# vita-epfl/CrowdNav

Hardware: AMD Instinct MI355X
Metric: env-steps/sec (whole node), 4096 envs x 5 humans, ORCA step (higher is better)
Workload: dtype f32 ORCA solve + f64 env step

## Files before the change

### crowdnav_amd/csrc/orca_device.h

```cpp
#pragma once
#include <hip/hip_runtime.h>

namespace cn {

constexpr int kWave = 64;
constexpr int kMaxNb = 10;
constexpr int kLineStride = kMaxNb + 1;
constexpr float kRvoEps = 0.00001f;
constexpr int kLazyCandFloat4 = (kWave / (kMaxNb - 1)) * ((kMaxNb - 1) + 4);

__device__ __forceinline__ void wave_lds_sync() {
    __builtin_amdgcn_fence(__ATOMIC_RELEASE, "wavefront");
    __builtin_amdgcn_wave_barrier();
    __builtin_amdgcn_fence(__ATOMIC_ACQUIRE, "wavefront");
}

__device__ __forceinline__ int opaque_tid() {
    int t = threadIdx.x;
    asm volatile("" : "+v"(t));
    return t;
}

struct OrcaParams {
    float neighbor_dist;
// ... 18 lines not shown
    const bool disc = overlap || (dot1 < 0.0f && dot1 * dot1 > rsum_sq * wlen_sq);
    const float root = sqrtf(disc ? wlen_sq : dist_sq - rsum_sq);
    const float inv = 1.0f / (disc ? root : dist_sq);
    const float nx = wx * inv, ny = wy * inv;
    const float kd = rsum * inv_t - root;
    const bool left = rpx * wy - rpy * wx > 0.0f;
    const float llx = (rpx * root - rpy * rsum) * inv, lly = (rpx * rsum + rpy * root) * inv;
    const float lrx = -((rpx * root + rpy * rsum) * inv), lry = -((-rpx * rsum + rpy * root) * inv);
    const float gx = left ? llx : lrx, gy = left ? lly : lry;
    const float dot2 = rvx * gx + rvy * gy;
    const float ldx = disc ? ny : gx;
    const float ldy = disc ? -nx : gy;
    const float ux = disc ? kd * nx : dot2 * gx - rvx;
    const float uy = disc ? kd * ny : dot2 * gy - rvy;
    return make_float4(svx + 0.5f * ux, svy + 0.5f * uy, ldx, ldy);
}

__device__ __forceinline__ void lp_start_point(float radius, float ox, float oy, float& rx, float& ry) {
    if (ox * ox + oy * oy > radius * radius) {
        const float inv = 1.0f / sqrtf(ox * ox + oy * oy);
        const float ux = ox * inv, uy = oy * inv;
        rx = ux * radius;
        ry = uy * radius;
    } else {
        rx = ox;
        ry = oy;
    }
}

template <int NJ>
__device__ __forceinline__ float4 lp_line_candidate(const float4 lk, const float4* prev, int k, float radius, float ox,
                                                    float oy, bool dir_opt) {
    const float px = lk.x, py = lk.y, dx = lk.z, dy = lk.w;
    const float dp = px * dx + py * dy;
    const float disc = (dp * dp + radius * radius) - (px * px + py * py);
    bool ok = !(disc < 0.0f);
    const float root = sqrtf(disc);
    float t_lo = -dp - root;
    float t_hi = -dp + root;
#pragma unroll
    for (int j = 0; j < NJ; ++j) {
        const float4 lj = prev[j];
        const bool use = j < k;
        const float den = dx * lj.w - dy * lj.z;
        const float num = lj.z * (py - lj.y) - lj.w * (px - lj.x);
        const bool parallel = fabsf(den) <= kRvoEps;
        const float t = num / den;
        ok = ok && !(use && parallel && num < 0.0f);
        const bool upper = use && !parallel && den >= 0.0f;
        const bool lower = use && !parallel && !(den >= 0.0f);
        t_hi = (upper && t < t_hi) ? t : t_hi;
        t_lo = (lower && t_lo < t) ? t : t_lo;
        ok = ok && !(t_lo > t_hi);
    }
    float t;
    if (dir_opt) {
        t = (ox * dx + oy * dy > 0.0f) ? t_hi : t_lo;
    } else {
        t = dx * (ox - px) + dy * (oy - py);
        t = (t < t_lo) ? t_lo : ((t > t_hi) ? t_hi : t);
    }
    return make_float4(px + t * dx, py + t * dy, ok ? 1.0f : 0.0f, 0.0f);
}

template <int MAXL>
__device__ __forceinline__ int lp_planar_scan(const float4* lines, const float4* cand, int n, float& rx, float& ry) {
    float4 lk[MAXL], ck[MAXL];
#pragma unroll
    for (int k = 0; k < MAXL; ++k) {
        lk[k] = lines[k];
        ck[k] = cand[k];
    }
    int fail = n;
#pragma unroll
    for (int k = 0; k < MAXL; ++k) {
        const float det = lk[k].z * (lk[k].y - ry) - lk[k].w * (lk[k].x - rx);
        const bool viol = (k < fail) & (det > 0.0f);
        const bool feasible = ck[k].z != 0.0f;
        rx = (viol & feasible) ? ck[k].x : rx;
        ry = (viol & feasible) ? ck[k].y : ry;
        fail = (viol & !feasible) ? k : fail;
    }
    return fail;
}

__device__ __forceinline__ int lp3_program_of(int m) { return m >= 6 ? 4 : (m >= 3 ? 3 : (m >= 1 ? 2 : 1)); }

__device__ __forceinline__ float4 lp3_project(const float4 li, const float4 lj) {
    const float d = li.z * lj.w - li.w * lj.z;
    const bool par = fabsf(d) <= kRvoEps;
    const bool same_dir = li.z * lj.z + li.w * lj.w > 0.0f;
    const float t = (lj.z * (li.y - lj.y) - lj.w * (li.x - lj.x)) / d;
    const float qx = par ? 0.5f * (li.x + lj.x) : li.x + t * li.z;
    const float qy = par ? 0.5f * (li.y + lj.y) : li.y + t * li.w;
    const float ex = lj.z - li.z, ey = lj.w - li.w;
    const float inv = 1.0f / sqrtf(ex * ex + ey * ey);
    const bool skip = par && same_dir;
    return make_float4(skip ? 0.0f : qx, skip ? 0.0f : qy, skip ? 0.0f : ex * inv, skip ? 0.0f : ey * inv);
}

__device__ __forceinline__ void lp3_scan(const float4* lines, const float4* proj, const float4* cand, int n, int begin,
                                         float radius, float& rx, float& ry) {
    float distance = 0.0f;
    float4 li[5];
#pragma unroll
    for (int i = 0; i < 5; ++i) li[i] = lines[i];
#pragma unroll
    for (int i = 0; i < 5; ++i) {
        float4 pk[4], ck[4];
#pragma unroll
        for (int k = 0; k < i; ++k) {
            pk[k] = proj[i * (i - 1) / 2 + k];
            ck[k] = cand[i * (i - 1) / 2 + k];
        }
        const float viol_i = li[i].z * (li[i].y - ry) - li[i].w * (li[i].x - rx);
        const bool active = (i >= begin) & (i < n) & (viol_i > distance);
        float r2x = -li[i].w * radius, r2y = li[i].z * radius;
        bool failed = false;
#pragma unroll
        for (int k = 0; k < i; ++k) {
            const float det = pk[k].z * (pk[k].y - r2y) - pk[k].w * (pk[k].x - r2x);
            const bool viol = !failed & (det > 0.0f);
            const bool feasible = ck[k].z != 0.0f;
            r2x = (viol & feasible) ? ck[k].x : r2x;
            r2y = (viol & feasible) ? ck[k].y : r2y;
            failed = failed | (viol & !feasible);
        }
        rx = (active & !failed) ? r2x : rx;
        ry = (active & !failed) ? r2y : ry;
        const float pen = li[i].z * (li[i].y - ry) - li[i].w * (li[i].x - rx);
        distance = active ? pen : distance;
    }
}

__device__ __forceinline__ float4 lp3_inner_program(const float4* proj, const float4* cand, int i, const float4 li, float radius) {
    const int base = i * (i - 1) / 2;
    float4 pk[4], ck[4];
#pragma unroll
    for (int k = 0; k < 4; ++k) {
        const int slot = base + k < 10 ? base + k : 9;
        pk[k] = proj[slot];
        ck[k] = cand[slot];
    }
    float r2x = -li.w * radius, r2y = li.z * radius;
    bool failed = false;
#pragma unroll
    for (int k = 0; k < 4; ++k) {
        const float det = pk[k].z * (pk[k].y - r2y) - pk[k].w * (pk[k].x - r2x);
        const bool viol = (k < i) & !failed & (det > 0.0f);
        const bool feasible = ck[k].z != 0.0f;
        r2x = (viol & feasible) ? ck[k].x : r2x;
        r2y = (viol & feasible) ? ck[k].y : r2y;
        failed = failed | (viol & !feasible);
    }
    return make_float4(r2x, r2y, failed ? 1.0f : 0.0f, 0.0f);
}
__device__ __forceinline__ void lp3_outer_scan(const float4* lines, const float4* prog, int n, int begin, float radius,
                                               float& rx, float& ry) {
    float4 li[5], pg[5];
#pragma unroll
    for (int i = 0; i < 5; ++i) {
        li[i] = lines[i];
        pg[i] = prog[i];
    }
    pg[0] = make_float4(-li[0].w * radius, li[0].z * radius, 0.0f, 0.0f);
    float distance = 0.0f;
// ... 157 lines not shown
        const float radius = sol[a].z;
        const float4 my = (l < n) ? lines[a * kLineStride + l] : make_float4(0.f, 0.f, 0.f, 0.f);
        float rx = r0.x, ry = r0.y, distance = 0.0f;
        int icur = need ? begin : n;
        while (true) {
            const bool cond = l >= icur && l < n && (my.z * (my.y - ry) - my.w * (my.x - rx) > distance);
            const unsigned long long m = __ballot(cond);
            if (m == 0ull) break;
            const unsigned gm = (unsigned)(m >> gbase) & kField;
            const bool act = gm != 0u;
            const int i = act ? __ffs(gm) - 1 : 0;
            const float4 li = lines[a * kLineStride + i];
            const float d = li.z * my.w - li.w * my.z;
            const bool par = fabsf(d) <= kRvoEps;
            const bool same_dir = li.z * my.z + li.w * my.w > 0.0f;
            const float t = (my.z * (li.y - my.y) - my.w * (li.x - my.x)) / d;
            const float qx = par ? 0.5f * (li.x + my.x) : li.x + t * li.z;
            const float qy = par ? 0.5f * (li.y + my.y) : li.y + t * li.w;
            const float ex = my.z - li.z, ey = my.w - li.w;
            const float inv = 1.0f / sqrtf(ex * ex + ey * ey);
            const float pz = ex * inv, pw = ey * inv;
            const bool valid = act && l < i && !(par && same_dir);
            const float ox = -li.w, oy = li.z;
            float r2x = ox * radius, r2y = oy * radius;
            int cur2 = 0;
            bool failed = false;
            while (true) {
                const bool viol = valid && l >= cur2 && (pz * (qy - r2y) - pw * (qx - r2x) > 0.0f);
                const unsigned long long m2 = __ballot(viol);
                if (m2 == 0ull) break;
                const unsigned gm2 = (unsigned)(m2 >> gbase) & kField;
                const bool act2 = gm2 != 0u;
                const int k = act2 ? __ffs(gm2) - 1 : 0;
                const float kx = __shfl(qx, gbase + k), ky = __shfl(qy, gbase + k);
                const float kz = __shfl(pz, gbase + k), kw = __shfl(pw, gbase + k);
                const float den = kz * pw - kw * pz;
                const float num = pz * (ky - qy) - pw * (kx - qx);
                const bool parallel = fabsf(den) <= kRvoEps;
                const float tk = num / den;
                const bool mine = act2 && valid && l < k;
                const bool bad = mine && parallel && num < 0.0f;
                const float c_hi = (mine && !parallel && den >= 0.0f) ? tk : inf;
                const float c_lo = (mine && !parallel && !(den >= 0.0f)) ? tk : -inf;
                const unsigned badm = (unsigned)(__ballot(bad) >> gbase) & kField;
                const float dp = kx * kz + ky * kw;
                const float disc = (dp * dp + radius * radius) - (kx * kx + ky * ky);
                bool ok = !(disc < 0.0f) && badm == 0u;
                const float root = sqrtf(disc);
                float t_lo = -dp - root;
                float t_hi = -dp + root;
#pragma unroll
                for (int j = 0; j < MAXL - 1; ++j) {
                    const float hj = __shfl(c_hi, gbase + j);
                    const float lj = __shfl(c_lo, gbase + j);
                    t_hi = (hj < t_hi) ? hj : t_hi;
                    t_lo = (t_lo < lj) ? lj : t_lo;
                }
                ok = ok && !(t_lo > t_hi);
                const float tt = (ox * kz + oy * kw > 0.0f) ? t_hi : t_lo;
                if (act2) {
                    if (ok) {
                        r2x = kx + tt * kz;
                        r2y = ky + tt * kw;
                        cur2 = k + 1;
                    } else {
                        failed = true;
                        cur2 = MAXL;
                    }
                }
            }
            if (act) {
                if (!failed) {
                    rx = r2x;
                    ry = r2y;
                }
                distance = li.z * (li.y - ry) - li.w * (li.x - rx);
                icur = i + 1;
            }
        }
        if (need && l == 0) res[a] = make_float4(rx, ry, r0.z, 0.0f);
    }
}

__device__ __forceinline__ float4 lp_line_candidate_pairs5(const float4* lq, int k, int lane, float radius, float ox, float oy) {
    const float inf = __builtin_inff();
    const float4 lk = lq[k];
    const int row0 = k == 0 ? 4 : k, j0 = k == 0 ? 2 : 0;
    const int row1 = k == 0 ? 4 : (k == 1 ? 3 : k), j1 = k == 0 ? 3 : (k == 1 ? 2 : 1);
    const bool own0 = k != 0, own1 = k >= 2;
    const float4 K0 = lq[row0], J0 = lq[j0], K1 = lq[row1], J1 = lq[j1];
    float hi_c[2], lo_c[2];
    bool bad_c[2];
#pragma unroll
    for (int s = 0; s < 2; ++s) {
        const float4 K = s ? K1 : K0, J = s ? J1 : J0;
        const float den = K.z * J.w - K.w * J.z;
        const float num = J.z * (K.y - J.y) - J.w * (K.x - J.x);
        const bool parallel = fabsf(den) <= kRvoEps;
        const float t = num / den;
        bad_c[s] = parallel && num < 0.0f;
        hi_c[s] = (!parallel && den >= 0.0f) ? t : inf;
        lo_c[s] = (!parallel && !(den >= 0.0f)) ? t : -inf;
    }
    float hi_o = own0 ? hi_c[0] : inf, lo_o = own0 ? lo_c[0] : -inf;
    bool bad_o = own0 && bad_c[0];
    float hi_h = own0 ? inf : hi_c[0], lo_h = own0 ? -inf : lo_c[0];
    bool bad_h = !own0 && bad_c[0];
    hi_o = (own1 && hi_c[1] < hi_o) ? hi_c[1] : hi_o;
    lo_o = (own1 && lo_o < lo_c[1]) ? lo_c[1] : lo_o;
    bad_o = bad_o || (own1 && bad_c[1]);
    hi_h = (!own1 && hi_c[1] < hi_h) ? hi_c[1] : hi_h;
    lo_h = (!own1 && lo_h < lo_c[1]) ? lo_c[1] : lo_h;
    bad_h = bad_h || (!own1 && bad_c[1]);
    const int src = lane - (k == 3 ? 2 : (k == 4 ? 4 : 0));
    const float hi_r = __shfl(hi_h, src), lo_r = __shfl(lo_h, src);
    const int bad_r = __shfl(bad_h ? 1 : 0, src);
    const bool has = k >= 3;
    const float px = lk.x, py = lk.y, dx = lk.z, dy = lk.w;
    const float dp = px * dx + py * dy;
    const float disc = (dp * dp + radius * radius) - (px * px + py * py);
    bool ok = !(disc < 0.0f);
    const float root = sqrtf(disc);
    float t_lo = -dp - root;
    float t_hi = -dp + root;
    t_hi = (hi_o < t_hi) ? hi_o : t_hi;
    t_lo = (t_lo < lo_o) ? lo_o : t_lo;
    t_hi = (has && hi_r < t_hi) ? hi_r : t_hi;
    t_lo = (has && t_lo < lo_r) ? lo_r : t_lo;
    ok = ok && !bad_o && !(has && bad_r != 0) && !(t_lo > t_hi);
    float t = dx * (ox - px) + dy * (oy - py);
    t = (t < t_lo) ? t_lo : ((t > t_hi) ? t_hi : t);
    return make_float4(px + t * dx, py + t * dy, ok ? 1.0f : 0.0f, 0.0f);
}

__device__ __forceinline__ float4 lp_line_candidate_pairs9(const float4 lk, const float4* prow, float4* bpart, int l, bool live,
                                                           float radius, float ox, float oy) {
    const float px = lk.x, py = lk.y, dx = lk.z, dy = lk.w;
    const float dp = px * dx + py * dy;
    const float disc = (dp * dp + radius * radius) - (px * px + py * py);
    bool ok = !(disc < 0.0f);
    const float root = sqrtf(disc);
    float t_lo = -dp - root;
    float t_hi = -dp + root;
    const float inf = __builtin_inff();
    const bool helper = l < 4;
    const float4 hk = prow[helper ? 8 - l : l];
    float hi_own = inf, lo_own = -inf, hi_help = inf, lo_help = -inf;
    bool bad_own = false, bad_help = false;
#pragma unroll
    for (int s = 0; s < 4; ++s) {
        const bool own = !helper || s < l;
        const float4 lj = prow[own ? s : 4 + s - l];
        const float kx = own ? px : hk.x, ky = own ? py : hk.y, kdx = own ? dx : hk.z, kdy = own ? dy : hk.w;
        const float den = kdx * lj.w - kdy * lj.z;
        const float num = lj.z * (ky - lj.y) - lj.w * (kx - lj.x);
        const bool parallel = fabsf(den) <= kRvoEps;
        const float t = num / den;
        const bool bad = parallel && num < 0.0f;
        const bool upper = !parallel && den >= 0.0f;
        const bool lower = !parallel && !(den >= 0.0f);
        hi_own = (own && upper && t < hi_own) ? t : hi_own;
        lo_own = (own && lower && lo_own < t) ? t : lo_own;
        bad_own = bad_own || (own && bad);
        hi_help = (!own && upper && t < hi_help) ? t : hi_help;
        lo_help = (!own && lower && lo_help < t) ? t : lo_help;
        bad_help = bad_help || (!own && bad);
    }
    if (live && helper) bpart[3 - l] = make_float4(hi_help, lo_help, bad_help ? 1.0f : 0.0f, 0.0f);
    wave_lds_sync();
    const bool has_help = l >= 5;
    const float4 hb = bpart[has_help ? l - 5 : 0];
    t_hi = (hi_own < t_hi) ? hi_own : t_hi;
    t_lo = (t_lo < lo_own) ? lo_own : t_lo;
    t_hi = (has_help && hb.x < t_hi) ? hb.x : t_hi;
    t_lo = (has_help && t_lo < hb.y) ? hb.y : t_lo;
    ok = ok && !bad_own && !(has_help && hb.z != 0.0f) && !(t_lo > t_hi);
    const float t = (ox * dx + oy * dy > 0.0f) ? t_hi : t_lo;
    return make_float4(px + t * dx, py + t * dy, ok ? 1.0f : 0.0f, 0.0f);
}

template <int MAXL, bool GROUP_ROWS = false>
__device__ __forceinline__ void lp_relaxed_lazy(const float4* lines, float4* proj, float4* cand, const int* count,
                                                const float4* sol, float4* res, const int* todo, int n_todo, int threads) {
    constexpr int W = MAXL - 1, G = kWave / W;
    constexpr unsigned kField = (1u << W) - 1u;
    const int tid = opaque_tid();
    const int wl = tid & (kWave - 1);
    const int g = wl / W, l = wl - g * W;
    const int gbase = g * W;
    const int waves = (threads + kWave - 1) / kWave;
    float4* const crow = cand + ((tid / kWave) * G + (g < G ? g : 0)) * W;
    float4* const bpart = cand + (size_t)waves * G * W + ((tid / kWave) * G + (g < G ? g : 0)) * 4;
#ifdef CN_PHASE_TIMING
    unsigned long long pt_rounds = 0ull, pt_hand = 0ull;
    const unsigned long long pt_t0 = __builtin_readcyclecounter();
#endif
    for (int chunk = tid / kWave; chunk * G < n_todo; chunk += waves) {
        const int hand_end = waves == 1 ? n_todo : (chunk * G + G < n_todo ? chunk * G + G : n_todo);
        int next = chunk * G + G;
        bool live = false, need = false, tail = false;
        int a = 0, n = 0, icur = 0;
        float radius = 0.0f, rx = 0.0f, ry = 0.0f, r0z = 0.0f, distance = 0.0f;
        float4 my = make_float4(0.f, 0.f, 0.f, 0.f), last = my;
        float4* prow = proj;
        const auto take = [&](int idx) {
            live = g < G && idx < hand_end;
            a = live ? todo[idx] : 0;
            const float4 r0 = res[a];
            n = live ? count[a] : 0;
            const int begin = __float_as_int(r0.z);
            need = live && begin < n;
            radius = sol[a].z;
            my = (l < n) ? lines[a * kLineStride + l] : make_float4(0.f, 0.f, 0.f, 0.f);
            tail = l == W - 1 && W < n;
            last = tail ? lines[a * kLineStride + W] : make_float4(0.f, 0.f, 0.f, 0.f);
// ... 74 lines not shown
```

### crowdnav_amd/csrc/rollout_fused.h

```cpp
#pragma once
#include "rollout_kernels.h"

namespace cn {

constexpr int kFusedMaxNC = 5;

template <typename T>
__device__ __forceinline__ T in_vgpr(T x) {
    asm volatile("" : "+v"(x));
    return x;
}

__device__ __forceinline__ void stage_agent(const Params& P, const Smem& s, const Lane& L, const AgentRegs& r,
                                            double human_safety, float4* kin) {
    if (L.lane >= P.nA) return;
    kin[L.lane] = make_float4((float)r.px, (float)r.py, (float)r.vx, (float)r.vy);
    s.posd[L.lane] = make_double2(r.px, r.py);
    s.rad[L.lane] = r.rad;
    s.hview[L.lane] = (float)(r.rad + 0.01 + human_safety);
}

__device__ __forceinline__ void preferred_velocity(const AgentRegs& r, float max_speed, bool solve, float4& sol, float4& start) {
    const double gdx = r.gx - r.px, gdy = r.gy - r.py;
    const double speed = norm2(gdx, gdy);
    const float pref_x = (float)(speed > 1.0 ? gdx / speed : gdx);
    const float pref_y = (float)(speed > 1.0 ? gdy / speed : gdy);
    sol = make_float4(pref_x, pref_y, max_speed, solve ? 1.0f : 0.0f);
    float sx, sy;
    lp_start_point(max_speed, pref_x, pref_y, sx, sy);
    start = make_float4(sx, sy, 0.0f, 0.0f);
}

#define CN_FUSED_SYNC() wave_lds_sync()



struct PairRow {
    int my_info, my_slot, xbase;
};
__device__ __forceinline__ PairRow pair_row_of(const Params& P, const Smem& s, int lane) {
    PairRow pr{0, P.nA, 0};
    if (lane < P.pairs) {
        pr.my_info = s.pinfo[lane];
        const int c = (pr.my_info >> 16) & 0xff;
        pr.xbase = (lane - c) * 4;
        pr.my_slot = ((pr.my_info >> 24) & 1) ? ((pr.my_info >> 8) & 0xff) : P.nA;
    }
    return pr;
}

__device__ __forceinline__ float pair_rsum(const Smem& s, const PairRow& pr) {
    const int q = pr.my_info & 0xff, ol = (pr.my_info >> 8) & 0xff;
    const float* view = ((pr.my_info >> 25) & 1) ? s.rview : s.hview;
    return view[q] + view[ol];
}

template <typename Mid>
__device__ __forceinline__ void fused_pair_body(const Params& P, const Smem& s, const PairRow& pr, float range_sq, float rsum,
                                                const float4 me, const float4 other, Mid&& mid) {
    const int my_info = pr.my_info;
    const int q = my_info & 0xff, c = (my_info >> 16) & 0xff;
    const float odx = me.x - other.x, ody = me.y - other.y;
    const float mine = odx * odx + ody * ody;
    uint32_t vbk[kFusedMaxNC];
#pragma unroll
    for (int k = 0; k < kFusedMaxNC; ++k) {
        const uint32_t got = (uint32_t)__builtin_amdgcn_ds_bpermute(pr.xbase + 4 * k, (int)__float_as_uint(mine));
        vbk[k] = k < P.NC ? got : 0x7f800000u;
    }
    int rank = 0, within = 0;
    {
        const uint32_t mb = __float_as_uint(mine), rb = __float_as_uint(range_sq);
        uint32_t before = 0u, inside = 0u;
#pragma unroll
        for (int k = 0; k < kFusedMaxNC; ++k) {
            const uint32_t vb = vbk[k];
            const uint32_t tie = (uint32_t)(k - c) >> 31;
            before = __builtin_amdgcn_alignbit(before, vb - mb - tie, 31);
            inside = __builtin_amdgcn_alignbit(inside, vb - rb, 31);
        }
        within = __popc(inside);
        rank = __popc(before & inside);
    }
    mid();
    if (c == 0) s.count[q] = within < P.orca.max_neighbors ? within : P.orca.max_neighbors;
    if (mine < range_sq && rank < P.orca.max_neighbors)
        s.lines[q * kLineStride + rank] =
            make_half_plane(P.orca, me.x, me.y, me.z, me.w, other.x, other.y, other.z, other.w, rsum);
}
template <typename Mid>
__device__ __forceinline__ void fused_pair_phase(const Params& P, const Smem& s, const PairRow& pr, float range_sq, float rsum,
                                                 Mid&& mid) {
    const float4 me = s.kin[pr.my_info & 0xff];
    const float4 other = s.kin[pr.my_slot];
    fused_pair_body(P, s, pr, range_sq, rsum, me, other, mid);
}

template <int MAXL>
__device__ __forceinline__ void fused_candidates(const Params& P, const Smem& s, int lane) {
    if (lane < P.nA * MAXL) {
        const int q = lane / MAXL, k = lane - q * MAXL;
        const float4 so = s.sol[q];
        const float4* lq = s.lines + q * kLineStride;
        s.cand2[q * kLineStride + k] = lp_line_candidate_pairs5(lq, k, lane, so.z, so.x, so.y);
    }
}

__device__ __forceinline__ void split_barrier() {
    asm volatile("s_waitcnt lgkmcnt(0)\n\ts_barrier" ::: "memory");
}

struct Lp3Item {
    int a, m, i, base;
    bool item;
    float4 li, lj;
    float radius;
};
template <int MAXL>
__device__ __forceinline__ Lp3Item lp3_item_of(const Smem& s, int lane, unsigned long long mask) {
    constexpr int kPairs = MAXL * (MAXL - 1) / 2;
    Lp3Item it;
    const int t = lane / kPairs;
    it.m = lane - t * kPairs;
    it.a = 0;
    unsigned long long rest = mask;
#pragma unroll
    for (int u = 0; u < kWave / kPairs; ++u) {
        const int bit = rest ? __ffsll((long long)rest) - 1 : 0;
        it.a = (u == t) ? bit : it.a;
        rest &= rest - 1ull;
    }
    it.item = lane < (int)__popcll(mask) * kPairs;
    it.i = lp3_program_of(it.m), it.base = it.i * (it.i - 1) / 2;
    const float4* la = s.lines + it.a * kLineStride;
    it.li = la[it.i], it.lj = la[it.m - it.base];
    it.radius = s.sol[it.a].z;
    return it;
}
template <int MAXL>
__device__ __forceinline__ void lp3_head(const Smem& s, const Lp3Item& it) {
    const float4 pr = lp3_project(it.li, it.lj);
    if (it.item) s.proj[it.a * kLineStride + it.m] = pr;
    CN_FUSED_SYNC();
    if (it.item) {
        const float4* pa = s.proj + it.a * kLineStride + it.base;
        s.cand3[it.a * kLineStride + it.m] =
            lp_line_candidate<MAXL - 2>(pa[it.m - it.base], pa, it.m - it.base, it.radius, -it.li.w, it.li.z, true);
    }
}

template <int MAXL>
__device__ __forceinline__ bool split_has_head(unsigned int pred, int u, int n_steps) {
    return pred != 0u && __popc(pred) * (MAXL * (MAXL - 1) / 2) <= kWave && u < n_steps;
}

struct NoOp {
    __device__ __forceinline__ void operator()() const {}
};
template <int MAXL, int BASE_PRIO = 0, typename AfterScan = NoOp>
__device__ __forceinline__ unsigned long long fused_solve(const Params& P, const Smem& s, int lane, bool solve, float& rx,
                                                          float& ry, PhaseClock* clk, unsigned long long have = 0ull,
                                                          AfterScan&& after_scan = NoOp{}) {
    (void)P, (void)clk;
    rx = 0.0f, ry = 0.0f;
    int n = 0, fail = 0;
    if (solve) {
        n = s.count[lane];
        const float4 start = s.res[lane];
        rx = start.x, ry = start.y;
        fail = lp_planar_scan<MAXL>(s.lines + lane * kLineStride, s.cand2 + lane * kLineStride, n, rx, ry);
    }
    CN_TICK(clk, 3);
    const bool need = solve && fail < n;
    const unsigned long long nm = __ballot(need);
#ifdef CN_PHASE_TIMING
    if (clk) clk->acc[9] += __popcll(nm);
#endif
    after_scan();
    if (nm == 0ull) __builtin_amdgcn_s_setprio(BASE_PRIO);
    if (nm != 0ull) {
        __builtin_amdgcn_s_setprio(3);
        constexpr int kPairs = MAXL * (MAXL - 1) / 2;
        const int n_todo = __popcll(nm);
        bool one_pass_done = false;
        if (n_todo * kPairs <= kWave) {
            const Lp3Item it = lp3_item_of<MAXL>(s, lane, nm);
            const bool item = it.item;
            const int a = it.a, i = it.i, m = it.m, base = it.base;
            const float4 li = it.li;
            const float radius = it.radius;
            const bool hit = (nm & ~have) == 0ull;
            if (!hit) {
                lp3_head<MAXL>(s, it);
                CN_FUSED_SYNC();
            }
            if (item && m == base)
                s.cand2[a * kLineStride + i] = lp3_inner_program(s.proj + a * kLineStride, s.cand3 + a * kLineStride, i, li, radius);
            CN_FUSED_SYNC();
            if (need)
                lp3_outer_scan(s.lines + lane * kLineStride, s.cand2 + lane * kLineStride, n, fail, s.sol[lane].z, rx, ry);
            one_pass_done = true;
        } else {
            if (need) s.todo[__popcll(nm & ((1ull << lane) - 1ull))] = lane;
            CN_FUSED_SYNC();
            const int items = n_todo * kPairs;
            for (int p = lane; p < items; p += kWave) {
                const int t = p / kPairs, m = p - t * kPairs;
                const int a = s.todo[t];
                const int i = lp3_program_of(m), j = m - i * (i - 1) / 2;
                const float4* la = s.lines + a * kLineStride;
                s.proj[a * kLineStride + m] = lp3_project(la[i], la[j]);
            }
            CN_FUSED_SYNC();
            for (int p = lane; p < items; p += kWave) {
                const int t = p / kPairs, m = p - t * kPairs;
                const int a = s.todo[t];
                const int i = lp3_program_of(m), base = i * (i - 1) / 2;
                const float4 li = s.lines[a * kLineStride + i];
                const float4* pa = s.proj + a * kLineStride + base;
                s.cand3[a * kLineStride + m] = lp_line_candidate<MAXL - 2>(pa[m - base], pa, m - base, s.sol[a].z, -li.w, li.z, true);
            }
            CN_FUSED_SYNC();
        }
        if (need && !one_pass_done)
            lp3_scan(s.lines + lane * kLineStride, s.proj + lane * kLineStride, s.cand3 + lane * kLineStride, n,
                     fail, s.sol[lane].z, rx, ry);
    }
    return nm;
}

struct StepConsts {
    double dt, limit, limit1, success, collision, ddist, dfactor, hsafety;
};
__device__ __forceinline__ StepConsts step_consts(const Params& P) {
    StepConsts K;
    K.dt = in_vgpr(P.dt), K.limit = in_vgpr(P.time_limit), K.limit1 = in_vgpr(P.time_limit - 1.0);
    K.success = in_vgpr(P.success_reward), K.collision = in_vgpr(P.collision_penalty);
    K.ddist = in_vgpr(P.discomfort_dist), K.dfactor = in_vgpr(P.discomfort_factor);
    K.hsafety = in_vgpr(P.human_safety);
    return K;
}

__device__ __forceinline__ double swept_distance(const AgentRegs& r, bool human, double2 rp, double act_x, double act_y,
                                                 double new_vx, double new_vy, double dt, double robot_rad) {
    const double x1 = r.px - rp.x, y1 = r.py - rp.y;
    const double wx = r.vx - act_x, wy = r.vy - act_y;
    const double x2 = x1 + wx * dt, y2 = y1 + wy * dt;
    const double sx = x2 - x1, sy = y2 - y1;
    double u = ((0.0 - x1) * sx + (0.0 - y1) * sy) / (sx * sx + sy * sy);
    u = (u > 1.0) ? 1.0 : ((u < 0.0) ? 0.0 : u);
    const bool degenerate = (sx == 0.0 && sy == 0.0);
    const double cx = degenerate ? 0.0 - x1 : (x1 + u * sx) - 0.0;
    const double cy = degenerate ? 0.0 - y1 : (y1 + u * sy) - 0.0;
    const double endx = r.px + new_vx * dt, endy = r.py + new_vy * dt;
    const double d = norm2(human ? cx : endx - r.gx, human ? cy : endy - r.gy);
    return human ? d - r.rad - robot_rad : d;
}

struct StepOutcome {
    double reward, dmin;
    int info;
    bool done;
};
__device__ __forceinline__ StepOutcome reduce_env(const Params& P, const Smem& s, int ebase, double gtime, const StepConsts& K) {
    const double goal_dist = s.closest[ebase];
    const double robot_rad = s.rad[ebase];
    double dmin = std::numeric_limits<double>::infinity();
    bool collision = false;
    for (int i = 1; i < P.A; ++i) {
        const double c = s.closest[ebase + i];
        const bool hit = c < 0.0;
        dmin = (!collision & !hit & (c < dmin)) ? c : dmin;
        collision = collision | hit;
    }
    const bool timeout = gtime >= K.limit1;
    const bool reaching = goal_dist < robot_rad;
    const bool danger = dmin < K.ddist;
    double reward = danger ? (dmin - K.ddist) * K.dfactor * K.dt : 0.0;
    int info = danger ? CN_DANGER : CN_NOTHING;
    reward = reaching ? K.success : reward, info = reaching ? CN_REACH_GOAL : info;
    reward = collision ? K.collision : reward, info = collision ? CN_COLLISION : info;
    reward = timeout ? 0.0 : reward, info = timeout ? CN_TIMEOUT : info;
    const bool done = timeout | collision | reaching;
    return StepOutcome{reward, dmin, info, done};
}


#ifdef CN_WAVE_TRACE
static __device__ unsigned long long cn_wave_trace[8192 * 6];
#endif

constexpr int kSplitOrcaPrio = 1;
constexpr int kAssistHead = 1;
#ifndef CN_SPLIT_HEAD_PRIO
#define CN_SPLIT_HEAD_PRIO 2
#endif
#ifndef CN_SPLIT_HEAD_TAIL_PRIO
#define CN_SPLIT_HEAD_TAIL_PRIO 1
#endif

#ifdef CN_SPLIT_PROBE
constexpr bool kSplitProbe = true;
static __device__ unsigned long long cn_split_probe[32];
#define SPLIT_PROBE_DECL()                                                                                   \
    unsigned long long sp_cnt[7] = {}, sp_wait[3] = {}, sp_w1[2] = {}, sp_n1[2] = {}, sp_dt = 0ull; \
    bool sp_prev_head = false
#define SPLIT_PROBE_WAIT(k, barrier)                                   \
    do {                                                               \
        const unsigned long long sp_t0 = __builtin_readcyclecounter(); \
        barrier;                                                       \
        sp_dt = __builtin_readcyclecounter() - sp_t0;                  \
        sp_wait[k] += sp_dt;                                           \
    } while (0)
#define SPLIT_PROBE_AFTER_1(word, head)                               \
    do {                                                               \
        if ((word) != 0u) sp_w1[0] += sp_dt, ++sp_n1[0];               \
        if (sp_prev_head) sp_w1[1] += sp_dt, ++sp_n1[1];               \
        sp_prev_head = (head);                                         \
    } while (0)
#define SPLIT_PROBE_STEP(ended, nm, head, pred)                                  \
    do {                                                                         \
        const bool sp_hit = (head) && (nm) != 0ull && ((nm) & ~(unsigned long long)(pred)) == 0ull; \
        ++sp_cnt[0], sp_cnt[1] += (ended) ? 1 : 0, sp_cnt[2] += (nm) != 0ull ? 1 : 0, sp_cnt[3] += (head) ? 1 : 0; \
        sp_cnt[4] += sp_hit ? 1 : 0, sp_cnt[5] += ((nm) != 0ull && !sp_hit) ? 1 : 0, sp_cnt[6] += ((head) && (nm) == 0ull) ? 1 : 0; \
    } while (0)
#define SPLIT_PROBE_FLUSH(lane, base)                                                        \
    do {                                                                                     \
        if ((lane) == 0) {                                                                   \
            if ((base) == 0)                                                                 \
                for (int k = 0; k < 7; ++k) atomicAdd(&cn_split_probe[k], sp_cnt[k]);        \
            for (int k = 0; k < 3; ++k) atomicAdd(&cn_split_probe[((base) ? 10 : 7) + k], sp_wait[k]); \
            for (int k = 0; k < 2; ++k) {                                                    \
                atomicAdd(&cn_split_probe[((base) ? 17 : 13) + k], sp_w1[k]);                \
                atomicAdd(&cn_split_probe[((base) ? 19 : 15) + k], sp_n1[k]);                \
            }                                                                                \
        }                                                                                    \
    } while (0)
#else
constexpr bool kSplitProbe = false;
#define SPLIT_PROBE_DECL() (void)0
#define SPLIT_PROBE_WAIT(k, barrier) barrier
#define SPLIT_PROBE_AFTER_1(word, head) (void)0
#define SPLIT_PROBE_STEP(ended, nm, head, pred) (void)0
#define SPLIT_PROBE_FLUSH(lane, base) (void)0
#endif

template <int MAXL, int ASSIST>
__device__ __forceinline__ void split_orca_wave(const Params& P, const Smem& s, int n_steps) {
    const int lane = (int)threadIdx.x - kWave;
    float2* const vel = reinterpret_cast<float2*>(s.act);
    const float range_sq = P.orca.neighbor_dist * P.orca.neighbor_dist;
    const double c_dt = in_vgpr(P.dt);
    split_barrier();
    __builtin_amdgcn_s_setprio(kSplitOrcaPrio);
    const PairRow pr = pair_row_of(P, s, lane);
    double px = 0.0, py = 0.0;
    float rx = 0.0f, ry = 0.0f;
    bool solved = false;
    float rsum = 0.0f;
    const int pq = pr.my_info & 0xff;
    SPLIT_PROBE_DECL();
    for (int u = 0;;) {
        SPLIT_PROBE_WAIT(0, split_barrier());
        const int2 words = make_int2(s.flag[0], ((ASSIST & kAssistHead) || kSplitProbe) ? s.flag[1] : 0);
        float4 me = s.kin[pq], other = s.kin[pr.my_slot];
        const bool ended = __builtin_amdgcn_readfirstlane(words.x) != 0;
        const unsigned int pred = ((ASSIST & kAssistHead) || kSplitProbe) ? (unsigned int)__builtin_amdgcn_readfirstlane(words.y) : 0u;
        if (!ended) ++u;
        if (u >= n_steps) {
            split_barrier();
            break;
        }
        const bool head = (ASSIST & kAssistHead) ? split_has_head<MAXL>(pred, u, n_steps) : false;
        SPLIT_PROBE_AFTER_1(pred, head);
        if (ended) {
            if (lane < P.nA) {
                const double2 p = s.posd[lane];
                px = p.x, py = p.y;
                s.kin[lane] = reinterpret_cast<const float4*>(s.d2)[lane];
            }
            CN_FUSED_SYNC();
            me = s.kin[pq], other = s.kin[pr.my_slot];
        }
        if (ended) rsum = pair_rsum(s, pr);
        if (lane < P.pairs) fused_pair_body(P, s, pr, range_sq, rsum, me, other, [] {});
        SPLIT_PROBE_WAIT(1, split_barrier());
        fused_candidates<MAXL>(P, s, lane);
        CN_FUSED_SYNC();
        if (ended) solved = lane < P.nA && s.sol[lane < P.nA ? lane : 0].w != 0.0f;
        const unsigned long long nm = fused_solve<MAXL, kSplitOrcaPrio>(P, s, lane, solved, rx, ry, nullptr, head ? pred : 0u, [&] {
            if (head) SPLIT_PROBE_WAIT(2, split_barrier());
        });
        if (lane < P.nA) vel[lane] = make_float2(rx, ry);
        if (((ASSIST & kAssistHead) || kSplitProbe) && lane == 0) s.flag[1] = (int)nm;
        if (solved) {
            px = px + (double)rx * c_dt;
            py = py + (double)ry * c_dt;
            s.kin[lane] = make_float4((float)px, (float)py, rx, ry);
        }
        SPLIT_PROBE_STEP(ended, nm, head, pred);
    }
    SPLIT_PROBE_FLUSH(lane, 0);
}

template <bool HEADLINE, bool SPLIT = false, int ASSIST = 0>
__global__ __launch_bounds__((SPLIT ? 2 : 1) * kWave, (SPLIT ? 4 : HEADLINE ? 3 : 1)) void rollout_fused_kernel(
    Params P_in, const StateView* Sd, const int* ring_filled_in, RolloutView R, int n_steps, const double* ext_action) {
    static_assert(HEADLINE || !SPLIT, "the two-wave kernel exists for the headline geometry only");
    static_assert(SPLIT || ASSIST == 0, "the env wave assists an ORCA wave: two-wave kernel only");
#ifdef CN_WAVE_TRACE
    const unsigned long long wt_entry = __builtin_amdgcn_s_memrealtime();
    unsigned long long wt_fallbacks = 0ull, wt_ends = 0ull;
#endif
    constexpr int MAXL = 5;
    Params P = P_in;
    P.async_fill = 0;
    if (HEADLINE) {
        P.A = 6, P.NC = 5, P.E = 2, P.nA = 12, P.pairs = 60, P.threads = 64;
    }
    const Smem s = carve<MAXL>(P);
    if constexpr (SPLIT) {
        if (__builtin_amdgcn_readfirstlane((int)threadIdx.x) >= kWave) {
            split_orca_wave<MAXL, ASSIST>(P, s, n_steps);
            return;
        }
    }
    const Lane L = lane_of(P);
    AgentRegs r = {};
    float robot_max_speed = 0.0f;
    const bool robot = L.valid && L.a == 0;
    const cn_rollout_io* iop = R.io;
    double theta = 0.0;
    EpisodeBook ep = {};
    {
        const StateView S = *Sd;
        const cn_rollout_io io = *iop;
        const size_t gi = L.valid ? L.gi : 0;
        const int env = L.valid ? L.env : 0;
        const double2 p0 = S.pos[gi], v0 = S.vel[gi], g0 = S.goal[gi], q0 = S.rv[gi];
        const bool have = P.robot_orca ? S.rsim_valid[env] != 0 : false;
        const float rr_kept = P.robot_orca ? S.rsim_radius[gi] : 0.0f;
        const float ms_kept = P.robot_orca ? S.rsim_max_speed[env] : 0.0f;
        const double theta0 = S.theta[env];
        EpisodeBook ep0;
        CN_LOAD_EPISODE(P, ep0, S, io, ring_filled_in, env);
        if (L.valid) {
            r.px = p0.x, r.py = p0.y, r.vx = v0.x, r.vy = v0.y, r.gx = g0.x, r.gy = g0.y, r.rad = q0.x, r.vpref = q0.y;
            ep = ep0;
            if (L.a == 0) theta = theta0;
            if (P.robot_orca) {
                const float rr = have ? rr_kept : (float)(r.rad + 0.01 + P.robot_safety);
                if (!have) S.rsim_radius[L.gi] = rr;
                s.rview[L.lane] = rr;
                if (L.a == 0) {
                    robot_max_speed = have ? ms_kept : (float)r.vpref;
                    if (!have) S.rsim_max_speed[L.env] = robot_max_speed;
                }
            }
        }
    }
    build_pairs(P, s);

    if (L.valid && ep.state == kWaitingScenario && scenario_ready(P, *Sd, L.env, ep.ep_count, ep.ring_filled)) {
        load_from_ring(P, *Sd, L, ep.ep_count % P.ring_mod, r);
        ep.state = kRunning;
        ep.gtime = 0.0;
        theta = 1.5707963267948966;
    }
    unsigned int transitions = 0;
    for (int t = threadIdx.x; t < kMaxDiscount; t += P.threads) s.disc[t] = t < R.discount_len ? R.discount[t] : 0.0;
    CN_FUSED_SYNC();
    if (L.lane == 0) s.kin[P.nA] = make_float4(std::numeric_limits<float>::infinity(), std::numeric_limits<float>::infinity(), 0.0f, 0.0f);
    const PairRow pr = pair_row_of(P, s, L.lane);
    const StepConsts K = step_consts(P);
    float4* const kin_stage = SPLIT ? reinterpret_cast<float4*>(s.d2) : s.kin;
    stage_agent(P, s, L, r, K.hsafety, kin_stage);
    CN_FUSED_SYNC();

#ifdef CN_PHASE_TIMING
    PhaseClock clock = {};
    PhaseClock* clk = &clock;
// ... 37 lines not shown
                new_vx = m_robot ? act_x : (double)mine.x;
                new_vy = m_robot ? act_y : (double)mine.y;
                if (mirror ? m_running : running) {
                    r.px = r.px + new_vx * K.dt;
                    r.py = r.py + new_vy * K.dt;
                    r.vx = new_vx;
                    r.vy = new_vy;
                }
            }
            if (u < n_steps && (L.lane < P.nA || mirror)) {
                const double gdx = r.gx - r.px, gdy = r.gy - r.py;
                const double speed = norm2(gdx, gdy);
                const double num = mirror ? gdy : gdx;
                const float pref = (float)(speed > 1.0 ? num / speed : num);
                const float pref_y = __uint_as_float(__builtin_amdgcn_permlane16_swap(__float_as_uint(pref), __float_as_uint(pref), false, false)[1]);
                if (L.lane < P.nA) {
                    const float max_speed = (L.a == 0) ? robot_max_speed : (float)r.vpref;
                    float sx, sy;
                    lp_start_point(max_speed, pref, pref_y, sx, sy);
                    s.sol[L.lane] = make_float4(pref, pref_y, max_speed, (running && (L.a > 0 || P.robot_orca)) ? 1.0f : 0.0f);
                    s.res[L.lane] = make_float4(sx, sy, 0.0f, 0.0f);
                }
            }
            SPLIT_PROBE_WAIT(1, split_barrier());
            if constexpr ((ASSIST & kAssistHead) != 0) {
                if (split_has_head<MAXL>(pred, u, n_steps)) {
                    __builtin_amdgcn_s_setprio(CN_SPLIT_HEAD_PRIO);
                    const Lp3Item it = lp3_item_of<MAXL>(s, L.lane, (unsigned long long)pred);
                    lp3_head<MAXL>(s, it);
                    __builtin_amdgcn_s_setprio(CN_SPLIT_HEAD_TAIL_PRIO);
                    SPLIT_PROBE_WAIT(2, split_barrier());
                }
            }
            bool ended = false;
            if (!skip) {
                const double2 rp = make_double2(__shfl(r0.px, L.ebase), __shfl(r0.py, L.ebase));
                if (L.valid) s.closest[L.lane] = swept_distance(r0, L.a > 0, rp, act_x, act_y, new_vx, new_vy, K.dt, s.rad[L.ebase]);
                CN_FUSED_SYNC();
                bool done = false;
                if (running) {
                    const double disc_t = s.disc[ep.cur_steps < kMaxDiscount ? ep.cur_steps : kMaxDiscount - 1];
                    const StepOutcome o = reduce_env(P, s, L.ebase, ep.gtime, K);
                    done = o.done;
                    ep.gtime += K.dt;
                    ++transitions;
                    CN_BOOK_TRANSITION(ep, ep.cur_steps < kMaxDiscount ? disc_t : 0.0, o.reward, o.info, o.dmin);
                    if (done) {
                        const cn_rollout_io io = *iop;
                        const StateView S = *Sd;
                        AgentRegs next = r;
                        load_from_ring(P, S, L, (ep.ep_count + 1) % P.ring_mod, next);
                        CN_END_EPISODE(P, S, io, L.env, L.a == 0, K.limit, o.info, ep, r = next; theta = 1.5707963267948966);
                    }
                }
                ended = __ballot(done) != 0ull;
            }
            if (ended) stage_agent(P, s, L, r, K.hsafety, kin_stage);
            if (ended) copy_to_mirror();
            if (L.lane == 0) s.flag[0] = ended ? 1 : 0;
            skip = ended;
            if constexpr ((ASSIST & kAssistHead) != 0 && CN_SPLIT_HEAD_TAIL_PRIO != 0) __builtin_amdgcn_s_setprio(0);
            if (u >= n_steps) break;
        }
        SPLIT_PROBE_FLUSH(L.lane, 10);
    }
    const int one_wave_steps = SPLIT ? 0 : n_steps;
    for (int step = 0; step < one_wave_steps; ++step) {
        const bool running = L.valid && ep.state == kRunning;
        const bool solve = running && (L.a > 0 || P.robot_orca);

        if (L.lane < P.pairs) {
            float4 sol4, start4;
            fused_pair_phase(P, s, pr, range_sq, pair_rsum(s, pr), [&] {
                preferred_velocity(r, (L.a == 0) ? robot_max_speed : (float)r.vpref, solve, sol4, start4);
            });
            if (L.lane < P.nA) {
                s.sol[L.lane] = sol4;
                s.res[L.lane] = start4;
            }
        }
        CN_FUSED_SYNC();
        CN_TICK(clk, 2);

        fused_candidates<MAXL>(P, s, L.lane);
        CN_FUSED_SYNC();

        float rx, ry;
        const bool fell_back = fused_solve<MAXL>(P, s, L.lane, solve, rx, ry, clk) != 0ull;
        (void)fell_back;
#ifdef CN_WAVE_TRACE
        if (fell_back) ++wt_fallbacks;
#endif
        CN_TICK(clk, 8);

        double act_x, act_y;
        if (P.robot_orca) {
            act_x = (double)__shfl(rx, L.ebase);
            act_y = (double)__shfl(ry, L.ebase);
        } else {
            act_x = L.valid ? ext_action[2 * (size_t)L.env] : 0.0;
            act_y = L.valid ? ext_action[2 * (size_t)L.env + 1] : 0.0;
        }
        const double new_vx = (L.a == 0) ? act_x : (double)rx;
        const double new_vy = (L.a == 0) ? act_y : (double)ry;

        if (L.valid)
            s.closest[L.lane] = swept_distance(r, L.a > 0, s.posd[L.ebase], act_x, act_y, new_vx, new_vy, K.dt, s.rad[L.ebase]);
        CN_FUSED_SYNC();
        CN_TICK(clk, 5);

        if (running) {
            const double disc_t = s.disc[ep.cur_steps < kMaxDiscount ? ep.cur_steps : kMaxDiscount - 1];
            const StepOutcome o = reduce_env(P, s, L.ebase, ep.gtime, K);
            const double reward = o.reward, dmin = o.dmin;
            const int info = o.info;
            const bool done = o.done;
            ep.gtime += K.dt;
            r.px = r.px + new_vx * K.dt;
            r.py = r.py + new_vy * K.dt;
            r.vx = new_vx;
            r.vy = new_vy;
            ++transitions;
            CN_BOOK_TRANSITION(ep, ep.cur_steps < kMaxDiscount ? disc_t : 0.0, reward, info, dmin);
#ifdef CN_WAVE_TRACE
            if (__ballot(done) != 0ull) ++wt_ends;
#endif
            if (done) {
                const cn_rollout_io io = *iop;
                CN_END_EPISODE(P, *Sd, io, L.env, L.a == 0, K.limit, info, ep,
                               load_from_ring(P, *Sd, L, ep.ep_count % P.ring_mod, r); theta = 1.5707963267948966);
            }
        }
        stage_agent(P, s, L, r, K.hsafety, kin_stage);
        CN_FUSED_SYNC();
        CN_TICK(clk, 7);
    }
#ifdef CN_PHASE_TIMING
    if ((threadIdx.x & (kWave - 1)) == 0) {
        unsigned long long total = 0ull;
        for (int k = 0; k < 10; ++k) {
            atomicAdd(&cn_phase_cycles[k], clock.acc[k]);
            if (k != 9) total += clock.acc[k];
        }
        atomicMax(&cn_phase_cycles[14], total);
        atomicMin(&cn_phase_cycles[13], total);
        atomicAdd(&cn_phase_cycles[15], 1ull);
    }
#endif

#ifdef CN_WAVE_TRACE
    const unsigned long long wt_exit = __builtin_amdgcn_s_memrealtime();
#endif
    const StateView S = *Sd;
    if (L.valid) CN_STORE_AGENT(S, L.gi, r);
    const cn_rollout_io io = *iop;
    if (robot) CN_STORE_EPISODE(P, S, io, L.env, ep, theta);
    rollout_epilogue(P, S, io, L, robot, transitions, ep.ep_count, reinterpret_cast<double*>(s.lines));
#ifdef CN_WAVE_TRACE
    if (threadIdx.x == 0 && blockIdx.x < 8192) {
        unsigned long long* w = cn_wave_trace + 6 * blockIdx.x;
        unsigned hw;
        asm volatile("s_getreg_b32 %0, hwreg(HW_REG_HW_ID)" : "=s"(hw));
        w[0] = wt_entry, w[1] = wt_loop, w[2] = wt_exit, w[3] = __builtin_amdgcn_s_memrealtime();
        w[4] = wt_fallbacks | (wt_ends << 32), w[5] = hw;
    }
#endif
}
// ... 3 lines not shown
```

Baseline: 1.530 billion.

## Branchless gated planar scan and hoisted candidate row indices in fused ORCA

```diff
diff --git a/crowdnav_amd/csrc/orca_device.h b/crowdnav_amd/csrc/orca_device.h
--- a/crowdnav_amd/csrc/orca_device.h
+++ b/crowdnav_amd/csrc/orca_device.h
@@ -124,6 +124,22 @@
         fail = (viol & !feasible) ? k : fail;
     }
     return fail;
+}
+
+template <int MAXL>
+__device__ __forceinline__ unsigned int lp_planar_scan_gated(const float4 (&lk)[MAXL], const float4 (&ck)[MAXL], float& rx,
+                                                             float& ry) {
+    unsigned int failed = 0u;
+#pragma unroll
+    for (int k = 0; k < MAXL; ++k) {
+        const float det = lk[k].z * (lk[k].y - ry) - lk[k].w * (lk[k].x - rx);
+        const float viol = __uint_as_float(__float_as_uint(det) | failed);
+        const bool take = viol > ck[k].z, stop = viol > ck[k].w;
+        rx = take ? ck[k].x : rx;
+        ry = take ? ck[k].y : ry;
+        failed = stop ? ~(unsigned int)k : failed;
+    }
+    return failed;
 }
 
 __device__ __forceinline__ int lp3_program_of(int m) { return m >= 6 ? 4 : (m >= 3 ? 3 : (m >= 1 ? 2 : 1)); }
@@ -447,55 +463,60 @@
     }
 }
 
-__device__ __forceinline__ float4 lp_line_candidate_pairs5(const float4* lq, int k, int lane, float radius, float ox, float oy) {
+struct LineRows5 {
+    float4 lk, K0, J0, K1, J1;
+};
+struct LineRowIdx5 {
+    int k, row0, j0, row1, j1;
+};
+__device__ __forceinline__ LineRowIdx5 lp_line_row_idx5(int k) {
+    return LineRowIdx5{k, k == 0 ? 4 : k, k == 0 ? 2 : 0, k == 0 ? 4 : (k == 1 ? 3 : k), k == 0 ? 3 : (k == 1 ? 2 : 1)};
+}
+__device__ __forceinline__ LineRows5 lp_line_rows5(const float4* lq, const LineRowIdx5& r) {
+    return LineRows5{lq[r.k], lq[r.row0], lq[r.j0], lq[r.row1], lq[r.j1]};
+}
+__device__ __forceinline__ float4 lp_line_candidate_pairs5(const LineRows5& rows, int k, int lane, int n, float radius, float ox,
+                                                           float oy) {
     const float inf = __builtin_inff();
-    const float4 lk = lq[k];
-    const int row0 = k == 0 ? 4 : k, j0 = k == 0 ? 2 : 0;
-    const int row1 = k == 0 ? 4 : (k == 1 ? 3 : k), j1 = k == 0 ? 3 : (k == 1 ? 2 : 1);
-    const bool own0 = k != 0, own1 = k >= 2;
-    const float4 K0 = lq[row0], J0 = lq[j0], K1 = lq[row1], J1 = lq[j1];
-    float hi_c[2], lo_c[2];
-    bool bad_c[2];
+    const float4 lk = rows.lk, K0 = rows.K0, J0 = rows.J0, K1 = rows.K1, J1 = rows.J1;
+    float hi_c[2], lo_c[2], nb_c[2];
 #pragma unroll
     for (int s = 0; s < 2; ++s) {
         const float4 K = s ? K1 : K0, J = s ? J1 : J0;
         const float den = K.z * J.w - K.w * J.z;
         const float num = J.z * (K.y - J.y) - J.w * (K.x - J.x);
-        const bool parallel = fabsf(den) <= kRvoEps;
         const float t = num / den;
-        bad_c[s] = parallel && num < 0.0f;
-        hi_c[s] = (!parallel && den >= 0.0f) ? t : inf;
-        lo_c[s] = (!parallel && !(den >= 0.0f)) ? t : -inf;
-    }
-    float hi_o = own0 ? hi_c[0] : inf, lo_o = own0 ? lo_c[0] : -inf;
-    bool bad_o = own0 && bad_c[0];
-    float hi_h = own0 ? inf : hi_c[0], lo_h = own0 ? -inf : lo_c[0];
-    bool bad_h = !own0 && bad_c[0];
-    hi_o = (own1 && hi_c[1] < hi_o) ? hi_c[1] : hi_o;
-    lo_o = (own1 && lo_o < lo_c[1]) ? lo_c[1] : lo_o;
-    bad_o = bad_o || (own1 && bad_c[1]);
-    hi_h = (!own1 && hi_c[1] < hi_h) ? hi_c[1] : hi_h;
-    lo_h = (!own1 && lo_h < lo_c[1]) ? lo_c[1] : lo_h;
-    bad_h = bad_h || (!own1 && bad_c[1]);
+        hi_c[s] = den > kRvoEps ? t : inf;
+        lo_c[s] = !(den >= -kRvoEps) ? t : -inf;
+        nb_c[s] = fabsf(den) <= kRvoEps ? num : 0.0f;
+    }
+    const float hi_f = hi_c[1] < hi_c[0] ? hi_c[1] : hi_c[0];
+    const float lo_f = lo_c[0] < lo_c[1] ? lo_c[1] : lo_c[0];
+    const float nb_f = nb_c[0] < 0.0f ? nb_c[0] : nb_c[1];
+    const bool k0 = k == 0, k1 = k == 1, has = k >= 3;
+    float hi_o = k1 ? hi_c[0] : hi_f, lo_o = k1 ? lo_c[0] : lo_f, nb_o = k1 ? nb_c[0] : nb_f;
+    hi_o = k0 ? inf : hi_o, lo_o = k0 ? -inf : lo_o, nb_o = k0 ? 0.0f : nb_o;
+    const float hi_h = k1 ? hi_c[1] : hi_f, lo_h = k1 ? lo_c[1] : lo_f, nb_h = k1 ? nb_c[1] : nb_f;
     const int src = lane - (k == 3 ? 2 : (k == 4 ? 4 : 0));
-    const float hi_r = __shfl(hi_h, src), lo_r = __shfl(lo_h, src);
-    const int bad_r = __shfl(bad_h ? 1 : 0, src);
-    const bool has = k >= 3;
+    const float hi_s = __shfl(hi_h, src), lo_s = __shfl(lo_h, src), nb_s = __shfl(nb_h, src);
+    const float hi_r = has ? hi_s : inf, lo_r = has ? lo_s : -inf, nb_r = has ? nb_s : 0.0f;
     const float px = lk.x, py = lk.y, dx = lk.z, dy = lk.w;
     const float dp = px * dx + py * dy;
     const float disc = (dp * dp + radius * radius) - (px * px + py * py);
-    bool ok = !(disc < 0.0f);
     const float root = sqrtf(disc);
     float t_lo = -dp - root;
     float t_hi = -dp + root;
     t_hi = (hi_o < t_hi) ? hi_o : t_hi;
     t_lo = (t_lo < lo_o) ? lo_o : t_lo;
-    t_hi = (has && hi_r < t_hi) ? hi_r : t_hi;
-    t_lo = (has && t_lo < lo_r) ? lo_r : t_lo;
-    ok = ok && !bad_o && !(has && bad_r != 0) && !(t_lo > t_hi);
+    t_hi = (hi_r < t_hi) ? hi_r : t_hi;
+    t_lo = (t_lo < lo_r) ? lo_r : t_lo;
+    const float nb = nb_o < 0.0f ? nb_o : nb_r;
+    const float neg = disc < 0.0f ? disc : nb;
+    const bool ok = !(neg < 0.0f) && !(t_lo > t_hi);
+    const float live = k < n ? 0.0f : inf;
     float t = dx * (ox - px) + dy * (oy - py);
     t = (t < t_lo) ? t_lo : ((t > t_hi) ? t_hi : t);
-    return make_float4(px + t * dx, py + t * dy, ok ? 1.0f : 0.0f, 0.0f);
+    return make_float4(px + t * dx, py + t * dy, ok ? live : inf, ok ? inf : live);
 }
 
 __device__ __forceinline__ float4 lp_line_candidate_pairs9(const float4 lk, const float4* prow, float4* bpart, int l, bool live,
diff --git a/crowdnav_amd/csrc/rollout_fused.h b/crowdnav_amd/csrc/rollout_fused.h
--- a/crowdnav_amd/csrc/rollout_fused.h
+++ b/crowdnav_amd/csrc/rollout_fused.h
@@ -96,13 +96,24 @@
     fused_pair_body(P, s, pr, range_sq, rsum, me, other, mid);
 }
 
+struct CandLane {
+    int q;
+    LineRowIdx5 rows;
+};
 template <int MAXL>
-__device__ __forceinline__ void fused_candidates(const Params& P, const Smem& s, int lane) {
+__device__ __forceinline__ CandLane cand_lane_of(int lane) {
+    const int q = lane / MAXL;
+    return CandLane{q, lp_line_row_idx5(lane - q * MAXL)};
+}
+template <int MAXL>
+__device__ __forceinline__ void fused_candidates(const Params& P, const Smem& s, int lane, const CandLane& cl) {
     if (lane < P.nA * MAXL) {
-        const int q = lane / MAXL, k = lane - q * MAXL;
+        const int q = cl.q, k = cl.rows.k;
+        const float4* lq = s.lines + q * kLineStride;
+        const LineRows5 rows = lp_line_rows5(lq, cl.rows);
         const float4 so = s.sol[q];
-        const float4* lq = s.lines + q * kLineStride;
-        s.cand2[q * kLineStride + k] = lp_line_candidate_pairs5(lq, k, lane, so.z, so.x, so.y);
+        const int n = s.count[q];
+        s.cand2[q * kLineStride + k] = lp_line_candidate_pairs5(rows, k, lane, n, so.z, so.x, so.y);
     }
 }
 
@@ -163,15 +174,21 @@
                                                           AfterScan&& after_scan = NoOp{}) {
     (void)P, (void)clk;
     rx = 0.0f, ry = 0.0f;
-    int n = 0, fail = 0;
+    unsigned int failed = 0u;
     if (solve) {
-        n = s.count[lane];
         const float4 start = s.res[lane];
+        float4 lk[MAXL], ck[MAXL];
+#pragma unroll
+        for (int k = 0; k < MAXL; ++k) {
+            lk[k] = s.lines[lane * kLineStride + k];
+            ck[k] = s.cand2[lane * kLineStride + k];
+        }
         rx = start.x, ry = start.y;
-        fail = lp_planar_scan<MAXL>(s.lines + lane * kLineStride, s.cand2 + lane * kLineStride, n, rx, ry);
+        failed = lp_planar_scan_gated<MAXL>(lk, ck, rx, ry);
     }
     CN_TICK(clk, 3);
-    const bool need = solve && fail < n;
+    const bool need = failed != 0u;
+    const int fail = (int)~failed;
     const unsigned long long nm = __ballot(need);
 #ifdef CN_PHASE_TIMING
     if (clk) clk->acc[9] += __popcll(nm);
@@ -198,7 +215,7 @@
                 s.cand2[a * kLineStride + i] = lp3_inner_program(s.proj + a * kLineStride, s.cand3 + a * kLineStride, i, li, radius);
             CN_FUSED_SYNC();
             if (need)
-                lp3_outer_scan(s.lines + lane * kLineStride, s.cand2 + lane * kLineStride, n, fail, s.sol[lane].z, rx, ry);
+                lp3_outer_scan(s.lines + lane * kLineStride, s.cand2 + lane * kLineStride, s.count[lane], fail, s.sol[lane].z, rx, ry);
             one_pass_done = true;
         } else {
             if (need) s.todo[__popcll(nm & ((1ull << lane) - 1ull))] = lane;
@@ -223,7 +240,7 @@
             CN_FUSED_SYNC();
         }
         if (need && !one_pass_done)
-            lp3_scan(s.lines + lane * kLineStride, s.proj + lane * kLineStride, s.cand3 + lane * kLineStride, n,
+            lp3_scan(s.lines + lane * kLineStride, s.proj + lane * kLineStride, s.cand3 + lane * kLineStride, s.count[lane],
                      fail, s.sol[lane].z, rx, ry);
     }
     return nm;
@@ -358,7 +375,13 @@
     float rx = 0.0f, ry = 0.0f;
     bool solved = false;
     float rsum = 0.0f;
+    static_assert(kLineStride > MAXL, "kin_none is the pad slot of a `lines` row");
+    float4* const kin_none = s.lines + (lane < P.nA ? lane : 0) * kLineStride + (kLineStride - 1);
+    float4* kin_dst = kin_none;
     const int pq = pr.my_info & 0xff;
+    CandLane cl = cand_lane_of<MAXL>(lane < P.nA * MAXL ? lane : 0);
+    cl.rows.row0 = in_vgpr(cl.rows.row0), cl.rows.j0 = in_vgpr(cl.rows.j0);
+    cl.rows.row1 = in_vgpr(cl.rows.row1), cl.rows.j1 = in_vgpr(cl.rows.j1);
     SPLIT_PROBE_DECL();
     for (int u = 0;;) {
         SPLIT_PROBE_WAIT(0, split_barrier());
@@ -385,18 +408,21 @@
         if (ended) rsum = pair_rsum(s, pr);
         if (lane < P.pairs) fused_pair_body(P, s, pr, range_sq, rsum, me, other, [] {});
         SPLIT_PROBE_WAIT(1, split_barrier());
-        fused_candidates<MAXL>(P, s, lane);
+        fused_candidates<MAXL>(P, s, lane, cl);
         CN_FUSED_SYNC();
-        if (ended) solved = lane < P.nA && s.sol[lane < P.nA ? lane : 0].w != 0.0f;
+        if (ended) {
+            solved = lane < P.nA && s.sol[lane < P.nA ? lane : 0].w != 0.0f;
+            kin_dst = solved ? s.kin + lane : kin_none;
+        }
         const unsigned long long nm = fused_solve<MAXL, kSplitOrcaPrio>(P, s, lane, solved, rx, ry, nullptr, head ? pred : 0u, [&] {
             if (head) SPLIT_PROBE_WAIT(2, split_barrier());
         });
-        if (lane < P.nA) vel[lane] = make_float2(rx, ry);
-        if (((ASSIST & kAssistHead) || kSplitProbe) && lane == 0) s.flag[1] = (int)nm;
-        if (solved) {
+        if (lane < P.nA) {
+            vel[lane] = make_float2(rx, ry);
+            if ((ASSIST & kAssistHead) || kSplitProbe) s.flag[1] = (int)nm;
             px = px + (double)rx * c_dt;
             py = py + (double)ry * c_dt;
-            s.kin[lane] = make_float4((float)px, (float)py, rx, ry);
+            *kin_dst = make_float4((float)px, (float)py, rx, ry);
         }
         SPLIT_PROBE_STEP(ended, nm, head, pred);
     }
@@ -600,7 +626,7 @@
         CN_FUSED_SYNC();
         CN_TICK(clk, 2);
 
-        fused_candidates<MAXL>(P, s, L.lane);
+        fused_candidates<MAXL>(P, s, L.lane, cand_lane_of<MAXL>(L.lane < P.nA * MAXL ? L.lane : 0));
         CN_FUSED_SYNC();
 
         float rx, ry;
```

After: 1.529 billion. About the same (-0.0%).
